# jihun1998/AO

Hardware: AMD Instinct MI355X
Metric: points/sec fwd+bwd PTv2m2 S3DIS (higher is better)
Workload: dtype fp32

## Files before the change

ao_amd/csrc/gva_wgrad_tile.hip:

```cpp
#include <algorithm>
#include <cstdlib>

#include "gva_common.h"
#include "wgrad_job.h"

namespace gva {

typedef float wt_v4f __attribute__((ext_vector_type(4)));
__device__ __forceinline__ wt_v4f wt_mfma(float a, float b, wt_v4f c) { return __builtin_amdgcn_mfma_f32_16x16x4f32(a, b, c, 0, 0, 0); }

constexpr int WT_PG = 16 * 16 + 4;

template <int G, int C, int GB, int NCW>
struct WgradTileCfg {
    static constexpr int NGW = GB / 4, QB = GB / 4, GS = G / GB, CR = C / (16 * NCW);
    static_assert(GB % 4 == 0 && GB <= 16 && G % GB == 0 && C == 8 * G && C % (16 * NCW) == 0, "blocks of groups x ranges of channels");
    static constexpr size_t lds_floats = (size_t)NCW * GB * WT_PG + 4 * 4 * 64;
};

template <int G, int C, int GB, int NCW>
__device__ __forceinline__ void wp2_wgrad_tile_body(const dense::WgradJob &J, const int bx, const int gs, const int cr, float *lds) {
    using K = WgradTileCfg<G, C, GB, NCW>;
    constexpr int NGW = K::NGW, QB = K::QB, PG = WT_PG;
    float *sA = lds;
// ... 100 lines not shown
        for (int gi = 0; gi < NGW; ++gi)
#pragma unroll
            for (int ck = 0; ck < NCW; ++ck) {
                const float *src = sA + (ck * GB + wid + 4 * gi) * PG + q * 16 + l15;
#pragma unroll
                for (int ks = 0; ks < 4; ++ks) accW[gi][ck] = wt_mfma(cur.goA[gi][ks], src[ks * 64], accW[gi][ck]);
            }
        __syncthreads();
    }
    float *rec = J.part + (size_t)bx * J.rec;
    if (q < 2) {
#pragma unroll
        for (int gi = 0; gi < NGW; ++gi)
#pragma unroll
            for (int ck = 0; ck < NCW; ++ck)
#pragma unroll
                for (int r = 0; r < 4; ++r)
                    rec[((size_t)(g0 + wid + 4 * gi) * 8 + 4 * q + r) * C + c0 + 16 * ck + l15] = accW[gi][ck][r];
    }
    if (bias_thread) rec[(size_t)G * 8 * C + o0 + tid] = bacc;
}

__global__ __launch_bounds__(256) void wp2_posrel_kernel_jobs(const dense::WgradJob *__restrict__ jobs, int njobs) {
    int j = 0;
    while (j + 1 < njobs && (long long)blockIdx.x >= jobs[j + 1].ldy) ++j;
    const dense::WgradJob &J = jobs[j];
    const long long e = ((long long)blockIdx.x - J.ldy) * 256 + threadIdx.x;
    if (e >= (long long)J.n * 16) return;
    const float *__restrict__ coord = (const float *)J.aux[0];
    const int *__restrict__ idx = (const int *)J.aux[1];
    const long long pt = e >> 4;
    const int sid = idx[e];
    const long long ss = sid >= 0 ? sid : 0;
    const float x = coord[3 * ss] - coord[3 * pt], y = coord[3 * ss + 1] - coord[3 * pt + 1], z = coord[3 * ss + 2] - coord[3 * pt + 2];
    ((float4 *)J.mX[0])[e] = sid >= 0 ? make_float4(x, y, z, 0.f) : make_float4(0.f, 0.f, 0.f, 0.f);
}

__device__ __forceinline__ void wp2_wgrad_tile_dispatch(const dense::WgradJob &J, int local, float *lds) {
    const int NS = J.chunks, GS = J.tiles;
    const int bx = local % NS, rest = local / NS, gs = rest % GS, cr = rest / GS;
    switch (J.batch) {
        case 12: wp2_wgrad_tile_body<12, 96, 12, 3>(J, bx, gs, cr, lds); break;
        case 24: wp2_wgrad_tile_body<24, 192, 12, 4>(J, bx, gs, cr, lds); break;
        case 48: wp2_wgrad_tile_body<48, 384, 12, 4>(J, bx, gs, cr, lds); break;
        default: wp2_wgrad_tile_body<64, 512, 16, 4>(J, bx, gs, cr, lds); break;
    }
}

__global__ __launch_bounds__(256, 2) void wp2_wgrad_tile_kernel(dense::WgradJob J) {
    extern __shared__ float4 wt_lds4[];
    wp2_wgrad_tile_dispatch(J, (int)blockIdx.x, (float *)wt_lds4);
}

__global__ __launch_bounds__(256, 2) void wp2_wgrad_tile_kernel_jobs(const dense::WgradJob *__restrict__ jobs, int njobs) {
    extern __shared__ float4 wt_lds4[];
    int j = 0;
    while (j + 1 < njobs && (int)blockIdx.x >= jobs[j + 1].wg0) ++j;
    const dense::WgradJob &J = jobs[j];
    wp2_wgrad_tile_dispatch(J, (int)blockIdx.x - J.wg0, (float *)wt_lds4);
}

constexpr size_t WT_LDS_BYTES = sizeof(float) * std::max({WgradTileCfg<12, 96, 12, 3>::lds_floats, WgradTileCfg<24, 192, 12, 4>::lds_floats,
                                                          WgradTileCfg<48, 384, 12, 4>::lds_floats, WgradTileCfg<64, 512, 16, 4>::lds_floats});

}

int gva_wgrad_tile_supported(int k, int c, int g) {
    return k == 16 && ((g == 12 && c == 96) || (g == 24 && c == 192) || (g == 48 && c == 384) || (g == 64 && c == 512));
}

size_t gva_wgrad_tile_plan(dense::WgradJob *J, int max_splits) {
    const int g = J->batch, c = J->cin;
    const int gb = g == 64 ? 16 : 12, ncw = g == 12 ? 3 : 4;
    const int tiles = (J->n + 15) / 16;
    J->tiles = g / gb;
    J->tiles_i = c / (16 * ncw);
    J->chunks = std::max(1, std::min({tiles / 6, 48, std::max(1, max_splits)}));
    J->chunk = (tiles + J->chunks - 1) / J->chunks * 16;
    J->rec = g * (8 * c + 8);
    J->wgs = J->chunks * J->tiles * J->tiles_i;
    J->has_pb = 1;
    J->count = 0;
    J->cout = 8;
    J->gw = gb;
    return (size_t)J->chunks * J->rec;
}

static bool wgrad_tile_configure() {
    static const bool ok = hipFuncSetAttribute((const void *)gva::wp2_wgrad_tile_kernel, hipFuncAttributeMaxDynamicSharedMemorySize,
                                               (int)gva::WT_LDS_BYTES) == hipSuccess &&
                           hipFuncSetAttribute((const void *)gva::wp2_wgrad_tile_kernel_jobs, hipFuncAttributeMaxDynamicSharedMemorySize,
                                               (int)gva::WT_LDS_BYTES) == hipSuccess;
    return ok;
}

int gva_wgrad_tile_launch_one(const dense::WgradJob &J, hipStream_t st) {
    if (!wgrad_tile_configure()) return PTV2_ERR_LAUNCH;
    hipLaunchKernelGGL(gva::wp2_wgrad_tile_kernel, dim3((unsigned)J.wgs), dim3(256), gva::WT_LDS_BYTES, st, J);
    return PTV2_OK;
}

int gva_wgrad_tile_launch_jobs(const dense::WgradJob *table, int njobs, int wgs, int pos_wgs, hipStream_t st) {
    if (!wgrad_tile_configure()) return PTV2_ERR_LAUNCH;
    if (pos_wgs > 0) hipLaunchKernelGGL(gva::wp2_posrel_kernel_jobs, dim3((unsigned)pos_wgs), dim3(256), 0, st, table, njobs);
    hipLaunchKernelGGL(gva::wp2_wgrad_tile_kernel_jobs, dim3((unsigned)wgs), dim3(256), gva::WT_LDS_BYTES, st, table, njobs);
    return PTV2_OK;
}
```

ao_amd/csrc/internal.h:

```cpp
#pragma once

struct GvaPlan;
namespace gva {
struct FoldWFwdArgs; struct FoldWBwdArgs; struct PtvDrop;
struct AttnIn; struct AttnFwdOut; struct AttnBwdIn; struct AttnBwdOut;
struct LogitsIn; struct LogitsOut; struct LogitsBwdIn; struct LogitsBwdOut;
}
namespace dense { struct WgradJob; struct BnTileSet; }

void ptv2_profile_scope(int which, int end, int ring_entry, int ring_size);
int rows_gemm_record_rows(int m, int n, int k);
void ptv2_gemm_allow_rb16(int on);
size_t bn_tiles_floats_rb(int n, int c, int rb);
int bn_tiles_finalize_rb(int n, int c, const dense::BnTileSet &S, float eps, float momentum, void *stream);
int bn_tiles_finalize_pair(int n, int c, const dense::BnTileSet (&S)[2], float eps, float momentum, void *stream);
int bn_tiles_apply_residual(int n, int c, const dense::BnTileSet &S, float eps, float momentum, const float *x,
                            const float *residual, const float *rowscale, float *y, void *stream);
int bn_tiles_apply_relu(int n, int c, const dense::BnTileSet &S, float eps, float momentum, const float *x, float *y, void *stream);
int skinny_linear_forward_pair(int n, int cin, int cout, const float *const *x, const float *W, const float *const *xsc,
                               const float *const *xsh, float *const *y, void *stream);
void ptv2_skinny_bn_arm(int n, int c, const float *const *x, const float *const *gy, const float *const *mean,
                        const float *const *rstd, const float *const *gamma, const float *const *beta, int relu, void *workspace,
                        size_t workspace_bytes);
void ptv2_skinny_bn_disarm(void);
struct PtvSkinnyBnScope {
    PtvSkinnyBnScope() = default;
    ~PtvSkinnyBnScope() { ptv2_skinny_bn_disarm(); }
    PtvSkinnyBnScope(const PtvSkinnyBnScope &) = delete;
    PtvSkinnyBnScope &operator=(const PtvSkinnyBnScope &) = delete;
};
int skinny_backward_pair_bn_reduce(int n, int cin, int cout, const float *const *gy, const float *W, float *const *gx,
                                   void *stream);
int ptv2_skinny_bn_take_records(int n, int c, const float *part, const float *const *gy);
extern "C" int linear_wgrad_strided_rowscale(int n, int cout, int cin, int batch, const float *gY, long long ldy, long long sy,
                                             const float *X, long long ldx, long long sx, float *dW, float *db,
                                             const float *rowscale, long long lds_s, int *weighted, void *workspace,
                                             size_t workspace_bytes, void *stream);
int gva_wp2_wgrad_recompute(int n, int k, int c, int g, const gva::AttnIn &I, const gva::AttnBwdIn &X, float *dW, float *db,
                            void *workspace, size_t workspace_bytes, void *stream);
int ptv2_blocks_fold_forward(int count, const ptv2_block *blocks, void *stream);
int gva_fold_forward_batched(int count, const ptv2_gva_block *blocks, void *stream);
int gva_block_forward_stats(const ptv2_gva_block *B, float *out_stats, int *stats_done, void *workspace, size_t workspace_bytes,
                            void *stream);
void ptv2_gva_set_prefolded(int on);
size_t ptv2_gva_fold_scratch_floats(int c, int g);
void ptv2_gva_set_fold_scratch(float *p);
int ptv2_gva_flush_folds(void *stream);
void ptv2_gva_drop_folds();
int gva_logits_forward_fold(const GvaPlan &P, int n, int k, int c, int g, const gva::LogitsIn &I, const gva::LogitsOut &O,
                            const gva::FoldWFwdArgs &F, void *workspace, size_t workspace_bytes, void *stream);
int gva_fwd_point_supported(int k, int c, int g);
int gva_fwd_point_max_n();
int gva_fwd_point_launch(int n, int k, int c, int g, const gva::AttnIn &I, const gva::AttnFwdOut &O, void *stream);
int gva_fwd_tile_supported(int k, int c, int g);
int gva_fwd_tile_launch(int n, int k, int c, int g, const gva::AttnIn &I, const gva::AttnFwdOut &O, void *stream);
int gva_peb_forward_stats(int n, int c, int g, const gva::AttnIn &I, const gva::AttnFwdOut &O, int *stats_done, void *stream);
int gva_aggregate_forward(const GvaPlan &P, int n, int k, int c, int g, const gva::AttnIn &I, const gva::AttnFwdOut &O,
                          void *stream);
int gva_aggregate_backward(const GvaPlan &P, int n, int k, int c, int g, const gva::AttnIn &I, const gva::AttnBwdIn &X,
                           const gva::AttnBwdOut &O, void *workspace, size_t workspace_bytes, void *stream);
int gva_logits_backward_foldw(const GvaPlan &P, int n, int k, int c, int g, const gva::LogitsIn &I, const gva::LogitsBwdIn &X,
                              const gva::FoldWBwdArgs &F, const gva::LogitsBwdOut &O, void *workspace, size_t workspace_bytes,
                              void *stream);
int gva_logits_bwd_fused_supported(int k, int c, int g);
int gva_logits_bwd_fused_launch(int n, int k, int c, int g, const gva::LogitsIn &I, const gva::LogitsBwdIn &X,
                                const gva::FoldWBwdArgs &F, float *gWt, float *part, size_t part_floats_avail,
                                const gva::LogitsBwdOut &O, hipStream_t st);
int gva_logits_fwd_mfma_supported(int k, int c, int g);
int gva_logits_fwd_mfma_launch(int n, int k, int c, int g, const gva::LogitsIn &I, const gva::LogitsOut &O, float *part,
                               const gva::FoldWFwdArgs &F, hipStream_t st);
int gva_bwd_point_supported(int k, int c, int g);
int gva_bwd_point_local(int k, int c, int g);
size_t gva_bwd_point_part_floats(int c, int g);
int gva_bwd_point_launch(int n, int k, int c, int g, const gva::AttnIn &I, const gva::AttnBwdIn &X, const gva::AttnBwdOut &O,
                         float *part, size_t part_floats_avail, hipStream_t st, gva::PtvDrop drop);
int gva_softmax_point_launch(int n, int k, int g, const gva::AttnIn &I, const gva::AttnFwdOut &O, hipStream_t st,
                             gva::PtvDrop drop);
int gva_logits_point_launch(int n, int k, int c, int g, const gva::LogitsIn &I, const gva::LogitsOut &O, float *part,
                            const gva::FoldWFwdArgs &F, hipStream_t st);
int gva_logits_params_point_launch(int n, int k, int c, int g, const gva::LogitsIn &I, const float *gWt, float *part,
                                   int max_blocks, int *nblk_out, hipStream_t st);
int gva_bwd_tile_supported(int k, int c, int g);
size_t gva_bwd_tile_part_floats(int n, int c, int g);
int gva_bwd_tile_launch(int n, int k, int c, int g, const gva::AttnIn &I, const gva::AttnBwdIn &X, const gva::AttnBwdOut &O,
                        float *part, size_t part_floats_avail, gva::PtvDrop drop, hipStream_t st);
int gva_wgrad_tile_supported(int k, int c, int g);
size_t gva_wgrad_tile_plan(dense::WgradJob *J, int max_splits);
int gva_wgrad_tile_launch_one(const dense::WgradJob &J, hipStream_t st);
int gva_wgrad_tile_launch_jobs(const dense::WgradJob *table, int njobs, int wgs, int pos_wgs, hipStream_t st);
```

ao_amd/csrc/wgrad.hip:

```cpp
#include <vector>

#include "dense_common.h"
#include "wgrad_job.h"

namespace dense {

using f32x4 = __attribute__((ext_vector_type(4))) float;
constexpr int WG_MT = 3, WG_TILE = 16 * WG_MT, WG_CHUNK = 256, WG_CHUNK_MIN = 128;

template <bool BF16>
__device__ __forceinline__ void wgrad_direct_tile(const int n, const int cout, const int cin, const int tiles_i,
                                                  const float *__restrict__ A, const long long ldy,
                                                  const float *__restrict__ B, const long long ldx, float *__restrict__ part,
                                                  const bool part_b, const int batch, const float *__restrict__ xs,
                                                  const float *__restrict__ xh, const int chunk, const int bx, const int by,
                                                  const int bz) {
    __shared__ float sRed[TPB / WAVE][WG_MT * WG_MT * 4 + WG_MT][WAVE + 1];
    const int lane = threadIdx.x & 63, wid = threadIdx.x >> 6;
    const int to = (by / tiles_i) * WG_TILE, ti = (by % tiles_i) * WG_TILE;
    const long long r0 = (long long)bx * chunk;
    const long long r1 = (r0 + chunk) < (long long)n ? (r0 + chunk) : (long long)n;
    const int lr = lane >> 4, lc = lane & 15;
    f32x4 acc[WG_MT][WG_MT];
    float bsum[WG_MT];
#pragma unroll
    for (int m = 0; m < WG_MT; ++m) {
        bsum[m] = 0.f;
#pragma unroll
        for (int t = 0; t < WG_MT; ++t) acc[m][t] = (f32x4){0.f, 0.f, 0.f, 0.f};
    }
    bool mo[WG_MT], mi[WG_MT];
    float xsc_[WG_MT], xsh_[WG_MT];
#pragma unroll
    for (int m = 0; m < WG_MT; ++m) {
        mo[m] = to + m * 16 + lc < cout;
        mi[m] = ti + m * 16 + lc < cin;
        xsc_[m] = (xs && mi[m]) ? xs[ti + m * 16 + lc] : 1.f;
        xsh_[m] = (xs && mi[m]) ? xh[ti + m * 16 + lc] : 0.f;
    }
    constexpr int U = 8;
    for (long long rb = r0 + 4 * wid; rb < r1; rb += 4 * (TPB / WAVE) * U) {
        float a[U][WG_MT], b[U][WG_MT];
#pragma unroll
        for (int u = 0; u < U; ++u) {
            const long long row = rb + (long long)u * 4 * (TPB / WAVE) + lr;
            const bool rok = row < r1;
#pragma unroll
            for (int m = 0; m < WG_MT; ++m) {
                a[u][m] = (rok && mo[m]) ? A[row * ldy + to + m * 16 + lc] : 0.f;
                b[u][m] = (rok && mi[m]) ? B[row * ldx + ti + m * 16 + lc] : 0.f;
            }
        }
        if (xs) {
#pragma unroll
            for (int u = 0; u < U; ++u)
#pragma unroll
                for (int m = 0; m < WG_MT; ++m) b[u][m] = fmaxf(__builtin_fmaf(b[u][m], xsc_[m], xsh_[m]), 0.f);
        }
        if constexpr (BF16) {
            ptv2_bf16x8 ab[WG_MT], bb[WG_MT];
#pragma unroll
            for (int m = 0; m < WG_MT; ++m) {
#pragma unroll
                for (int u = 0; u < U; ++u) {
                    bsum[m] += a[u][m];
                    ab[m][u] = (__bf16)a[u][m];
                    bb[m][u] = (__bf16)b[u][m];
                }
            }
#pragma unroll
            for (int m = 0; m < WG_MT; ++m)
#pragma unroll
                for (int t = 0; t < WG_MT; ++t)
                    acc[m][t] = __builtin_amdgcn_mfma_f32_16x16x32_bf16(ab[m], bb[t], acc[m][t], 0, 0, 0);
        } else {
#pragma unroll
            for (int u = 0; u < U; ++u)
#pragma unroll
                for (int m = 0; m < WG_MT; ++m) {
                    bsum[m] += a[u][m];
#pragma unroll
                    for (int t = 0; t < WG_MT; ++t)
                        acc[m][t] = __builtin_amdgcn_mfma_f32_16x16x4f32(a[u][m], b[u][t], acc[m][t], 0, 0, 0);
                }
        }
    }
#pragma unroll
    for (int m = 0; m < WG_MT; ++m) {
        float bs = bsum[m];
        bs += __shfl_xor(bs, 16, WAVE);
        bs += __shfl_xor(bs, 32, WAVE);
        sRed[wid][WG_MT * WG_MT * 4 + m][lane] = bs;
#pragma unroll
        for (int t = 0; t < WG_MT; ++t)
#pragma unroll
            for (int r = 0; r < 4; ++r) sRed[wid][(m * WG_MT + t) * 4 + r][lane] = acc[m][t][r];
    }
    __syncthreads();
    const size_t rec = (size_t)batch * cout * cin + (part_b ? (size_t)batch * cout : 0);
    float *p = part + (size_t)bx * rec + (size_t)bz * cout * cin;
    for (int e = threadIdx.x; e < WG_MT * WG_MT * 4 * WAVE; e += TPB) {
        const int q = e / WAVE, l = e - q * WAVE;
        const int mt = q / 4, r = q - mt * 4, m = mt / WG_MT, t = mt - m * WG_MT;
        const int o = to + m * 16 + (l >> 4) * 4 + r, i = ti + t * 16 + (l & 15);
        if (o < cout && i < cin) {
            float v = 0.f;
#pragma unroll
            for (int wv = 0; wv < TPB / WAVE; ++wv) v += sRed[wv][q][l];
            p[(size_t)o * cin + i] = v;
        }
    }
    if (part_b && ti == 0 && threadIdx.x < WG_TILE) {
        const int m = threadIdx.x >> 4, l = threadIdx.x & 15, o = to + threadIdx.x;
        if (o < cout) {
            float v = 0.f;
#pragma unroll
            for (int wv = 0; wv < TPB / WAVE; ++wv) v += sRed[wv][WG_MT * WG_MT * 4 + m][l];
            part[(size_t)bx * rec + (size_t)batch * cout * cin + (size_t)bz * cout + o] = v;
        }
    }
}

template <bool BF16>
__device__ __forceinline__ void wgrad_direct_job(const WgradJob &J, const int bx, const int by, const int bz) {
    const bool multi = J.count > 0;
    wgrad_direct_tile<BF16>(J.n, J.cout, J.cin, J.tiles_i, multi ? J.mgY[bz] : J.gY + (long long)bz * J.sy, J.ldy,
                            multi ? J.mX[bz] : J.X + (long long)bz * J.sx, J.ldx, J.part, J.has_pb != 0, J.batch,
                            multi ? J.mxsc[bz] : nullptr, multi ? J.mxsh[bz] : nullptr, J.chunk, bx, by, bz);
}
template <bool BF16>
__global__ __launch_bounds__(TPB) void linear_wgrad_kernel(WgradJob J) {
    wgrad_direct_job<BF16>(J, (int)blockIdx.x, (int)blockIdx.y, (int)blockIdx.z);
}

constexpr int WL_ROWS = 64;
template <int RS>
__device__ __forceinline__ void wgrad_lds_tile(const int n, const int cout, const int cin, const int tiles_i,
                                               const float *__restrict__ A, const long long ldy,
                                               const float *__restrict__ B, const long long ldx,
                                               float *__restrict__ part, const bool part_b, const int batch,
                                               const float *__restrict__ xs, const float *__restrict__ xh, const int chunk,
                                               const float *__restrict__ rowscale, const long long lds_s, const int bx,
                                               const int by, const int bz) {
    extern __shared__ float4 wl_lds4[];
    float *sA = (float *)wl_lds4;
    float *sB = sA + 2 * WL_ROWS * WG_TILE;
    const int tid = threadIdx.x, lane = tid & 63, wid = tid >> 6;
    const int to = (by / tiles_i) * WG_TILE, ti = (by % tiles_i) * WG_TILE;
    const long long r0 = (long long)bx * chunk;
    const long long r1 = (r0 + chunk) < (long long)n ? (r0 + chunk) : (long long)n;
    const int lr = lane >> 4, lc = lane & 15;
    f32x4 acc[WG_MT][WG_MT];
    float bsum[WG_MT];
#pragma unroll
    for (int m = 0; m < WG_MT; ++m) {
        bsum[m] = 0.f;
#pragma unroll
        for (int t = 0; t < WG_MT; ++t) acc[m][t] = (f32x4){0.f, 0.f, 0.f, 0.f};
    }
    float xsc_[WG_MT], xsh_[WG_MT];
#pragma unroll
    for (int m = 0; m < WG_MT; ++m) {
        const bool mi = ti + m * 16 + lc < cin;
        xsc_[m] = (xs && mi) ? xs[ti + m * 16 + lc] : 1.f;
        xsh_[m] = (xs && mi) ? xh[ti + m * 16 + lc] : 0.f;
    }
    constexpr int Q = WG_TILE / 4, SLOTS = WL_ROWS * Q / TPB;
    float4 ra[SLOTS], rb[SLOTS];
    float sn[4], sc_[4];
    auto fetch = [&](long long rs) {
#pragma unroll
        for (int j = 0; j < SLOTS; ++j) {
            const int f = tid + TPB * j, row = f / Q, c4 = (f - row * Q) * 4;
            const long long r = rs + row;
            ra[j] = ptv2_ld_or_zero((const float4 *)(A + r * ldy + to + c4), r < r1 && to + c4 < cout);
            rb[j] = ptv2_ld_or_zero((const float4 *)(B + r * ldx + ti + c4), r < r1 && ti + c4 < cin);
        }
        if constexpr (RS != 0) {
#pragma unroll
            for (int ks = 0; ks < 4; ++ks) {
                const long long r = rs + wid * 16 + ks * 4 + lr;
                sn[ks] = ptv2_ld_or_zero(rowscale + r * lds_s + bz, r < r1);
            }
        }
    };
// ... 51 lines not shown
        bs += __shfl_xor(bs, 16, WAVE);
        bs += __shfl_xor(bs, 32, WAVE);
        sRed[wid][WG_MT * WG_MT * 4 + m][lane] = bs;
#pragma unroll
        for (int t = 0; t < WG_MT; ++t)
#pragma unroll
            for (int r = 0; r < 4; ++r) sRed[wid][(m * WG_MT + t) * 4 + r][lane] = acc[m][t][r];
    }
    __syncthreads();
    const size_t rec = (size_t)batch * cout * cin + (part_b ? (size_t)batch * cout : 0);
    float *p = part + (size_t)bx * rec + (size_t)bz * cout * cin;
    for (int e = threadIdx.x; e < WG_MT * WG_MT * 4 * WAVE; e += TPB) {
        const int q = e / WAVE, l = e - q * WAVE;
        const int mt = q / 4, r = q - mt * 4, m = mt / WG_MT, t = mt - m * WG_MT;
        const int o = to + m * 16 + (l >> 4) * 4 + r, i = ti + t * 16 + (l & 15);
        if (o < cout && i < cin) {
            float v = 0.f;
#pragma unroll
            for (int wv = 0; wv < TPB / WAVE; ++wv) v += sRed[wv][q][l];
            p[(size_t)o * cin + i] = v;
        }
    }
    if (part_b && ti == 0 && threadIdx.x < WG_TILE) {
        const int m = threadIdx.x >> 4, l = threadIdx.x & 15, o = to + threadIdx.x;
        if (o < cout) {
            float v = 0.f;
#pragma unroll
            for (int wv = 0; wv < TPB / WAVE; ++wv) v += sRed[wv][WG_MT * WG_MT * 4 + m][l];
            part[(size_t)bx * rec + (size_t)batch * cout * cin + (size_t)bz * cout + o] = v;
        }
    }
}

template <int RS>
__device__ __forceinline__ void wgrad_lds_job(const WgradJob &J, const int bx, const int by, const int bz) {
    const bool multi = J.count > 0;
    wgrad_lds_tile<RS>(J.n, J.cout, J.cin, J.tiles_i, multi ? J.mgY[bz] : J.gY + (long long)bz * J.sy, J.ldy,
                       multi ? J.mX[bz] : J.X + (long long)bz * J.sx, J.ldx, J.part, J.has_pb != 0, J.batch,
                       multi ? J.mxsc[bz] : nullptr, multi ? J.mxsh[bz] : nullptr, J.chunk, J.rowscale, J.lds_s, bx, by, bz);
}
template <int RS>
__global__ __launch_bounds__(TPB) void linear_wgrad_lds_kernel(WgradJob J) {
    wgrad_lds_job<RS>(J, (int)blockIdx.x, (int)blockIdx.y, (int)blockIdx.z);
}

constexpr int WGRAD_PACK = 8;
struct WgradJobPack { WgradJob j[WGRAD_PACK]; };
static_assert(sizeof(WgradJobPack) + 16 <= 4096, "the table writer's argument block must fit the 4 KB kernarg segment");
__global__ void wgrad_jobs_write_kernel(WgradJobPack pack, int count, WgradJob *table) {
    if ((int)threadIdx.x < count) table[threadIdx.x] = pack.j[threadIdx.x];
}

template <int RS>
__global__ __launch_bounds__(TPB) void linear_wgrad_lds_kernel_jobs(const WgradJob *__restrict__ jobs, int njobs) {
    int j = 0;
    while (j + 1 < njobs && (int)blockIdx.x >= jobs[j + 1].wg0) ++j;
    const WgradJob &J = jobs[j];
    const int local = (int)blockIdx.x - J.wg0;
    const int rest = local / J.chunks;
    wgrad_lds_job<RS>(J, local % J.chunks, rest % J.tiles, rest / J.tiles);
}

constexpr int GRP_I = 8;
__device__ __forceinline__ void grouped_wgrad_tile(const int n, const int c, const int g, const int gw, const int chunk,
                                                   const float *__restrict__ gY, const float *__restrict__ X,
                                                   const float *__restrict__ sw, float *__restrict__ part, const int rec,
                                                   const int bx, const int bg) {
    extern __shared__ float4 grp_lds4[];
    const int q = c >> 2, units = gw * q, R = max(1, TPB / units);
    const int tid = threadIdx.x, rs = tid / units, u = tid - rs * units;
    const bool active = rs < R;
    const int gl = u / q, qi = u - gl * q, grp = bg * gw + gl;
    const bool live = active && grp < g;
    float4 acc[GRP_I];
    float bacc[GRP_I];
#pragma unroll
    for (int i = 0; i < GRP_I; ++i) { acc[i] = make_float4(0.f, 0.f, 0.f, 0.f); bacc[i] = 0.f; }
    const long long r0 = (long long)bx * chunk, r1 = (r0 + chunk) < (long long)n ? (r0 + chunk) : (long long)n;
    if (live) {
        const float *xa = X + (size_t)grp * c + 4 * qi;
        const float *ya = gY + (size_t)grp * GRP_I;
        const float *sa = sw + grp;
        const size_t xs = (size_t)g * c;
        constexpr int U = 4;
        long long r = r0 + rs;
        for (; r + (long long)(U - 1) * R < r1; r += (long long)U * R) {
            float4 a[U], y0[U], y1[U];
            float s[U];
#pragma unroll
            for (int t = 0; t < U; ++t) {
                const size_t rr = (size_t)(r + (long long)t * R);
                a[t] = *(const float4 *)(xa + rr * xs);
                y0[t] = *(const float4 *)(ya + rr * c);
                y1[t] = *(const float4 *)(ya + rr * c + 4);
                s[t] = qi == 0 ? sa[rr * g] : 0.f;
            }
#pragma unroll
            for (int t = 0; t < U; ++t) {
                const float y[GRP_I] = {y0[t].x, y0[t].y, y0[t].z, y0[t].w, y1[t].x, y1[t].y, y1[t].z, y1[t].w};
#pragma unroll
                for (int i = 0; i < GRP_I; ++i) {
                    acc[i].x = __builtin_fmaf(y[i], a[t].x, acc[i].x); acc[i].y = __builtin_fmaf(y[i], a[t].y, acc[i].y);
                    acc[i].z = __builtin_fmaf(y[i], a[t].z, acc[i].z); acc[i].w = __builtin_fmaf(y[i], a[t].w, acc[i].w);
                    bacc[i] = __builtin_fmaf(y[i], s[t], bacc[i]);
                }
            }
        }
        for (; r < r1; r += R) {
            const size_t rr = (size_t)r;
            const float4 a = *(const float4 *)(xa + rr * xs), y0 = *(const float4 *)(ya + rr * c), y1 = *(const float4 *)(ya + rr * c + 4);
            const float sv = qi == 0 ? sa[rr * g] : 0.f;
            const float y[GRP_I] = {y0.x, y0.y, y0.z, y0.w, y1.x, y1.y, y1.z, y1.w};
#pragma unroll
            for (int i = 0; i < GRP_I; ++i) {
                acc[i].x = __builtin_fmaf(y[i], a.x, acc[i].x); acc[i].y = __builtin_fmaf(y[i], a.y, acc[i].y);
                acc[i].z = __builtin_fmaf(y[i], a.z, acc[i].z); acc[i].w = __builtin_fmaf(y[i], a.w, acc[i].w);
                bacc[i] = __builtin_fmaf(y[i], sv, bacc[i]);
            }
        }
    }
    float4 *sAcc = grp_lds4;
    float *sB = (float *)(sAcc + (size_t)R * GRP_I * units);
    if (active) {
#pragma unroll
        for (int i = 0; i < GRP_I; ++i) {
            sAcc[((size_t)rs * GRP_I + i) * units + u] = acc[i];
            if (qi == 0) sB[((size_t)rs * GRP_I + i) * gw + gl] = bacc[i];
        }
    }
    __syncthreads();
    if (rs == 0 && grp < g) {
        float *p = part + (size_t)bx * rec;
#pragma unroll
        for (int i = 0; i < GRP_I; ++i) {
            float4 v = sAcc[(size_t)i * units + u];
            for (int t = 1; t < R; ++t) {
                const float4 w = sAcc[((size_t)t * GRP_I + i) * units + u];
                v.x += w.x; v.y += w.y; v.z += w.z; v.w += w.w;
            }
            *(float4 *)(p + ((size_t)grp * GRP_I + i) * c + 4 * qi) = v;
            if (qi == 0) {
                float b = sB[(size_t)i * gw + gl];
                for (int t = 1; t < R; ++t) b += sB[((size_t)t * GRP_I + i) * gw + gl];
                p[(size_t)g * GRP_I * c + (size_t)grp * GRP_I + i] = b;
            }
        }
    }
}
inline size_t grouped_lds_bytes(int c, int gw) {
    const int units = gw * (c >> 2), R = std::max(1, TPB / units);
    return sizeof(float4) * (size_t)R * GRP_I * units + sizeof(float) * (size_t)R * GRP_I * gw;
}
__global__ __launch_bounds__(TPB) void grouped_wgrad_kernel(WgradJob J) {
    const int bx = (int)blockIdx.x % J.chunks, bg = (int)blockIdx.x / J.chunks;
    grouped_wgrad_tile(J.n, J.cin, J.batch, J.gw, J.chunk, J.gY, J.X, J.rowscale, J.part, J.rec, bx, bg);
}
__global__ __launch_bounds__(TPB) void grouped_wgrad_kernel_jobs(const WgradJob *__restrict__ jobs, int njobs) {
    int j = 0;
    while (j + 1 < njobs && (int)blockIdx.x >= jobs[j + 1].wg0) ++j;
    const WgradJob &J = jobs[j];
    const int local = (int)blockIdx.x - J.wg0;
    grouped_wgrad_tile(J.n, J.cin, J.batch, J.gw, J.chunk, J.gY, J.X, J.rowscale, J.part, J.rec, local % J.chunks, local / J.chunks);
}

template <bool BF16>
__global__ __launch_bounds__(TPB) void linear_wgrad_kernel_jobs(const WgradJob *__restrict__ jobs, int njobs) {
    int j = 0;
    while (j + 1 < njobs && (int)blockIdx.x >= jobs[j + 1].wg0) ++j;
    const WgradJob &J = jobs[j];
    const int local = (int)blockIdx.x - J.wg0;
    const int rest = local / J.chunks;
    wgrad_direct_job<BF16>(J, local % J.chunks, rest % J.tiles, rest / J.tiles);
}

__global__ __launch_bounds__(256) void wgrad_jobs_finalize_kernel(const WgradJob *__restrict__ jobs, int njobs, int total) {
    __shared__ double s_sum[3][64];
    const int sidx = blockIdx.x * 256 + threadIdx.x;
    int j = 0;
    while (j + 1 < njobs && (int)blockIdx.x * 256 >= jobs[j + 1].fin0) ++j;
    const WgradJob &J = jobs[j];
    const int lanes = J.fin_lanes, local = sidx - J.fin0;
    const int rg = lanes == 1 ? 0 : (int)threadIdx.x >> 6;
    const int col = lanes == 1 ? local : (local >> 8) * 64 + ((int)threadIdx.x & 63);
    const int nblk = J.chunks;
    const size_t len = (size_t)J.rec;
    const float *part = J.part;
    const bool ok = col < J.rec;
    double a0 = 0.0, a1 = 0.0, a2 = 0.0, a3 = 0.0;
    if (ok) {
        int b = rg;
        for (; b + 3 * lanes < nblk; b += 4 * lanes) {
            a0 += (double)part[(size_t)b * len + col];
            a1 += (double)part[(size_t)(b + lanes) * len + col];
            a2 += (double)part[(size_t)(b + 2 * lanes) * len + col];
            a3 += (double)part[(size_t)(b + 3 * lanes) * len + col];
        }
        for (; b < nblk; b += lanes) a0 += (double)part[(size_t)b * len + col];
    }
    double acc = (a0 + a1) + (a2 + a3);
    if (lanes != 1) {
        if (rg > 0) s_sum[rg - 1][threadIdx.x & 63] = acc;
        __syncthreads();
        if (rg > 0) return;
        acc = (acc + s_sum[0][threadIdx.x]) + (s_sum[1][threadIdx.x] + s_sum[2][threadIdx.x]);
    }
    if (!ok) return;
    const float v = (float)acc;
    const int wlen = J.cout * J.cin, wtot = J.batch * wlen;
    if (J.count > 0) {
        if (col < wtot) {
            const int p = col / wlen;
            J.mdW[p][col - p * wlen] = v;
        } else {
            const int r = col - wtot, p = r / J.cout;
            if (J.mdb[p]) J.mdb[p][r - p * J.cout] = v;
        }
    } else if (col < wtot) {
        J.dW[col] = v;
    } else if (J.db) {
        J.db[col - wtot] = v;
    }
}

static bool wgrad_lds_ok(const void *a, long long ldy, long long sy, const void *b, long long ldx, long long sx) {
    return ((uintptr_t)a % 16 == 0) && ((uintptr_t)b % 16 == 0) && ldy % 4 == 0 && ldx % 4 == 0 && sy % 4 == 0 && sx % 4 == 0;
}
static bool wgrad_lds_shape_ok(int cout, int cin) { return cout % 4 == 0 && cin % 4 == 0; }
constexpr size_t WL_LDS_BYTES = sizeof(float) * std::max<size_t>(4 * (size_t)WL_ROWS * WG_TILE,
                                                                 (size_t)(TPB / WAVE) * (WG_MT * WG_MT * 4 + WG_MT) * (WAVE + 1));

}

using namespace dense;

extern "C" size_t dense_workspace_bytes(int n, int cout, int cin) {
    const size_t chunks = (size_t)(n + WG_CHUNK_MIN - 1) / WG_CHUNK_MIN + 1;
    const size_t wg = sizeof(float) * chunks * ((size_t)cout * cin + cout);
    const size_t bn = sizeof(float) * (size_t)MAX_BLK * 2 * (size_t)std::max(cout, cin);
    return ptv2_align256(std::max(wg, bn)) + 1024;
}

static int wg_chunk(int n, int tiles, bool filed = false) {
    const int target = filed ? 256 : 768;
    const int chunks = std::max(1, target / std::max(1, tiles));
    const long long rows = ((long long)n + chunks - 1) / chunks;
    long long chunk = std::max<long long>(WG_CHUNK, (rows + 127) / 128 * 128);
    if (tiles > 1) {
        int guard = 0;
        while ((((long long)n + chunk - 1) / chunk) % 8 == 0 && ((long long)n + chunk - 1) / chunk > 1 && guard++ < 16) chunk += 128;
    }
    return (int)std::min<long long>(chunk, 1 << 20);
}

namespace {
enum WgradForm { WF_LDS = 0, WF_LDS_RS, WF_DIRECT, WF_DIRECT_BF16, WF_GROUPED, WF_RECOMPUTE, WGRAD_FORMS };
constexpr int wgrad_kid(WgradForm f) {
    return f == WF_RECOMPUTE ? KID_WGRAD_TILE : f == WF_GROUPED ? KID_WGRAD_GROUPED : (f == WF_LDS || f == WF_LDS_RS) ? KID_WGRAD_LDS : KID_WGRAD;
}
struct WgradCall {
    WgradJob J;
    WgradForm form;
    double bytes;
    size_t posrel;
};

struct WgradDefer {
    bool active = false;
    bool armed = false;
    bool armed_rs = false;
    char *arena = nullptr;
    size_t cap = 0, used = 0;
    std::vector<WgradJob> jobs[WGRAD_FORMS];
    double bytes[WGRAD_FORMS] = {};
};
thread_local WgradDefer g_wdefer;
constexpr int WGRAD_MAX_JOBS = 64;
constexpr size_t WGRAD_TABLE_BYTES = ptv2_align256(sizeof(WgradJob) * WGRAD_MAX_JOBS);

bool may_file(bool rs) { return g_wdefer.active && (rs ? g_wdefer.armed_rs : g_wdefer.armed); }

bool wgrad_configure() {
    static const bool ok = [] {
        const void *kernels[4] = {(const void *)linear_wgrad_lds_kernel<0>, (const void *)linear_wgrad_lds_kernel<1>,
                                  (const void *)linear_wgrad_lds_kernel_jobs<0>, (const void *)linear_wgrad_lds_kernel_jobs<1>};
        bool all = true;
        for (const void *k : kernels)
            all = hipFuncSetAttribute(k, hipFuncAttributeMaxDynamicSharedMemorySize, (int)WL_LDS_BYTES) == hipSuccess && all;
        return all;
    }();
    return ok;
}
}

void ptv2_wgrad_defer_begin(void *arena, size_t bytes) {
    WgradDefer &D = g_wdefer;
    for (int f = 0; f < WGRAD_FORMS; ++f) { D.jobs[f].clear(); D.bytes[f] = 0.0; }
    D.armed = D.armed_rs = false;
    D.active = arena != nullptr && bytes > WGRAD_FORMS * WGRAD_TABLE_BYTES;
    D.arena = (char *)arena;
    D.cap = bytes;
    D.used = WGRAD_FORMS * WGRAD_TABLE_BYTES;
}
bool ptv2_wgrad_defer_active() { return g_wdefer.active; }
void ptv2_wgrad_defer_end() {
    g_wdefer.active = g_wdefer.armed = g_wdefer.armed_rs = false;
    for (auto &j : g_wdefer.jobs) j.clear();
}
void ptv2_wgrad_defer_arm(bool on) { g_wdefer.armed = on && g_wdefer.active; }
void ptv2_wgrad_defer_arm_rs(bool on) { g_wdefer.armed_rs = on && g_wdefer.active; }
bool ptv2_wgrad_defer_armed_rs() { return may_file(true); }
size_t ptv2_wgrad_defer_table_bytes() { return WGRAD_FORMS * WGRAD_TABLE_BYTES; }
float *ptv2_wgrad_defer_alloc(size_t floats) {
    WgradDefer &D = g_wdefer;
    const size_t bytes = ptv2_align256(sizeof(float) * floats);
    if (!D.active || D.used + bytes > D.cap) return nullptr;
    float *p = (float *)(D.arena + D.used);
    D.used += bytes;
    return p;
}
int ptv2_wgrad_defer_flush(void *stream) {
    WgradDefer &D = g_wdefer;
    if (!D.active) return PTV2_OK;
    hipStream_t st = (hipStream_t)stream;
    if (!wgrad_configure()) return PTV2_ERR_LAUNCH;
    for (int f = 0; f < WGRAD_FORMS; ++f) {
        const WgradForm form = (WgradForm)f;
        std::vector<WgradJob> &jobs = D.jobs[form];
        if (jobs.empty()) continue;
        WgradJob *table = (WgradJob *)(D.arena + (size_t)form * WGRAD_TABLE_BYTES);
        const int njobs = (int)jobs.size();
        const bool row_pieces = form == WF_GROUPED || form == WF_RECOMPUTE;
        std::stable_sort(jobs.begin(), jobs.end(), [row_pieces](const WgradJob &a, const WgradJob &b) {
            const long long wa = (long long)a.chunk * (row_pieces ? a.gw * a.cin : 1), wb = (long long)b.chunk * (row_pieces ? b.gw * b.cin : 1);
            return wa > wb;
        });
        int wgs = 0, fin = 0;
        long long pos_wgs = 0;
        bool pos_all = form == WF_RECOMPUTE;
        for (WgradJob &J : jobs) {
            if (form == WF_RECOMPUTE) {
                J.ldy = pos_wgs;
                pos_wgs += ((long long)J.n * 16 + 255) / 256;
                pos_all = pos_all && J.mX[0] != nullptr;
            }
            J.wg0 = wgs; J.fin0 = fin;
            J.fin_lanes = J.chunks > 32 ? 4 : 1;
            wgs += J.wgs;
            fin += J.fin_lanes == 1 ? (J.rec + 255) / 256 * 256 : (J.rec + 63) / 64 * 256;
        }
        for (int at = 0; at < njobs; at += WGRAD_PACK) {
            WgradJobPack pack;
            const int cnt = std::min(WGRAD_PACK, njobs - at);
            for (int i = 0; i < WGRAD_PACK; ++i) pack.j[i] = jobs[(size_t)std::min(at + i, njobs - 1)];
            hipLaunchKernelGGL(wgrad_jobs_write_kernel, dim3(1), dim3(64), 0, st, pack, cnt, table + at);
        }
        {
            PtvScopedTimer t(wgrad_kid(form), st, D.bytes[form]);
            const dim3 grid((unsigned)wgs), block(TPB);
            const WgradJob *tab = table;
            switch (form) {
                case WF_LDS: hipLaunchKernelGGL(linear_wgrad_lds_kernel_jobs<0>, grid, block, WL_LDS_BYTES, st, tab, njobs); break;
                case WF_LDS_RS: hipLaunchKernelGGL(linear_wgrad_lds_kernel_jobs<1>, grid, block, WL_LDS_BYTES, st, tab, njobs); break;
                case WF_DIRECT: hipLaunchKernelGGL(linear_wgrad_kernel_jobs<false>, grid, block, 0, st, tab, njobs); break;
                case WF_DIRECT_BF16: hipLaunchKernelGGL(linear_wgrad_kernel_jobs<true>, grid, block, 0, st, tab, njobs); break;
                case WF_GROUPED: {
                    size_t lds = 0;
                    for (const WgradJob &J : jobs) lds = std::max(lds, grouped_lds_bytes(J.cin, J.gw));
                    hipLaunchKernelGGL(grouped_wgrad_kernel_jobs, grid, block, lds, st, tab, njobs);
                    break;
                }
                default:
                    if (gva_wgrad_tile_launch_jobs(tab, njobs, wgs, pos_all ? (int)pos_wgs : 0, st) != PTV2_OK) return PTV2_ERR_LAUNCH;
            }
        }
        hipLaunchKernelGGL(wgrad_jobs_finalize_kernel, dim3((unsigned)((fin + 255) / 256)), dim3(256), 0, st,
                           (const WgradJob *)table, njobs, fin);
        jobs.clear();
        D.bytes[form] = 0.0;
    }
    PTV2_CHECK_LAUNCH();
    return PTV2_OK;
}

struct MapWgradMulti {
    float *dW[6], *db[6];
    int count, wlen, cout;
    explicit MapWgradMulti(const WgradJob &J) : count(J.count), wlen(J.cout * J.cin), cout(J.cout) {
        for (int i = 0; i < 6; ++i) { dW[i] = J.mdW[i]; db[i] = J.mdb[i]; }
    }
    __device__ void operator()(int e, double v) const {
        const int wtot = count * wlen;
        if (e < wtot) {
            const int b = e / wlen;
            dW[b][e - b * wlen] = (float)v;
        } else {
            const int r = e - wtot, b = r / cout;
            if (db[b]) db[b][r - b * cout] = (float)v;
        }
    }
};

namespace gva {
template <> struct RiderOf<MapWgradMulti> {
    static constexpr bool ok = true;
    static PtvRider make(const MapWgradMulti &m) {
        PtvRider r{};
        r.kind = RIDER_WGRADN;
        for (int i = 0; i < 6; ++i) { r.p[i] = i < m.count ? m.dW[i] : nullptr; r.p[6 + i] = i < m.count ? m.db[i] : nullptr; }
        r.i0 = m.wlen; r.i1 = m.cout; r.i2 = m.count;
        return r;
    }
};
}

static int wgrad_submit(WgradCall &C, bool file, void *workspace, size_t workspace_bytes, void *stream) {
    WgradDefer &D = g_wdefer;
    WgradJob &J = C.J;
    if (file && (int)D.jobs[C.form].size() < WGRAD_MAX_JOBS) {
        float *keep = ptv2_wgrad_defer_alloc((size_t)J.chunks * J.rec);
        float *pos = keep && C.posrel ? ptv2_wgrad_defer_alloc(C.posrel) : nullptr;
        if (keep && (pos || !C.posrel)) {
            J.part = keep;
            if (pos) J.mX[0] = pos;
            D.jobs[C.form].push_back(J);
            D.bytes[C.form] += C.bytes;
            return PTV2_OK;
        }
    }
    const size_t fit = workspace ? workspace_bytes / (sizeof(float) * (size_t)J.rec) : 0;
    if (C.form == WF_RECOMPUTE && fit >= 1 && fit < (size_t)J.chunks) (void)gva_wgrad_tile_plan(&J, (int)fit);
    if (fit < (size_t)J.chunks) return PTV2_ERR_WORKSPACE;
// ... 179 lines not shown
```

ao_amd/csrc/wgrad_job.h:

```cpp
#pragma once

namespace dense {

struct WgradJob {
    int n, cout, cin, tiles_i, tiles, batch, chunk, chunks;
    int wg0;
    int has_pb, count;
    int rec, fin0;
    int wgs, gw;
    int fin_lanes;
    long long ldy, sy, ldx, sx, lds_s;
    const float *gY, *X, *rowscale;
    float *part;
    const float *mgY[6], *mX[6], *mxsc[6], *mxsh[6];
    float *dW, *db, *mdW[6], *mdb[6];
    const void *aux[4];
};

}
```

Baseline: 12.84 million.

## Fold previous form's wgrad finalize blocks into next form's wgrad launch

When several wgrad forms are flushed, the finalize reduction for one form is prepended as extra blocks to the next form's wgrad kernel grid instead of being a separate launch. All job tables are written up front so the carried finalize can read them, and LDS is shared between the finalize and main paths. This cuts kernel launches and lets the small reduction overlap with the next GEMM-like work. The cost is a larger grid, an extra branch per block and more complex plan bookkeeping. It is gated by an env var (on by default) and a block-count cap.

```diff
diff --git a/ao_amd/csrc/gva_wgrad_tile.hip b/ao_amd/csrc/gva_wgrad_tile.hip
--- a/ao_amd/csrc/gva_wgrad_tile.hip
+++ b/ao_amd/csrc/gva_wgrad_tile.hip
@@ -176,12 +176,15 @@
     wp2_wgrad_tile_dispatch(J, (int)blockIdx.x, (float *)wt_lds4);
 }
 
-__global__ __launch_bounds__(256, 2) void wp2_wgrad_tile_kernel_jobs(const dense::WgradJob *__restrict__ jobs, int njobs) {
+__global__ __launch_bounds__(256, 2) void wp2_wgrad_tile_kernel_jobs(const dense::WgradJob *__restrict__ jobs, int njobs,
+                                                                     dense::WgradRide R) {
     extern __shared__ float4 wt_lds4[];
+    if (dense::wgrad_ride_block(R, (int)blockIdx.x, wt_lds4)) return;
+    const int bid = (int)blockIdx.x - R.fin_blocks;
     int j = 0;
-    while (j + 1 < njobs && (int)blockIdx.x >= jobs[j + 1].wg0) ++j;
+    while (j + 1 < njobs && bid >= jobs[j + 1].wg0) ++j;
     const dense::WgradJob &J = jobs[j];
-    wp2_wgrad_tile_dispatch(J, (int)blockIdx.x - J.wg0, (float *)wt_lds4);
+    wp2_wgrad_tile_dispatch(J, bid - J.wg0, (float *)wt_lds4);
 }
 
 constexpr size_t WT_LDS_BYTES = sizeof(float) * std::max({WgradTileCfg<12, 96, 12, 3>::lds_floats, WgradTileCfg<24, 192, 12, 4>::lds_floats,
@@ -224,9 +227,11 @@
     return PTV2_OK;
 }
 
-int gva_wgrad_tile_launch_jobs(const dense::WgradJob *table, int njobs, int wgs, int pos_wgs, hipStream_t st) {
+int gva_wgrad_tile_launch_jobs(const dense::WgradJob *table, int njobs, int wgs, int pos_wgs, const dense::WgradRide &R,
+                               hipStream_t st) {
     if (!wgrad_tile_configure()) return PTV2_ERR_LAUNCH;
     if (pos_wgs > 0) hipLaunchKernelGGL(gva::wp2_posrel_kernel_jobs, dim3((unsigned)pos_wgs), dim3(256), 0, st, table, njobs);
-    hipLaunchKernelGGL(gva::wp2_wgrad_tile_kernel_jobs, dim3((unsigned)wgs), dim3(256), gva::WT_LDS_BYTES, st, table, njobs);
+    hipLaunchKernelGGL(gva::wp2_wgrad_tile_kernel_jobs, dim3((unsigned)(R.fin_blocks + wgs)), dim3(256), gva::WT_LDS_BYTES, st, table,
+                       njobs, R);
     return PTV2_OK;
 }
diff --git a/ao_amd/csrc/internal.h b/ao_amd/csrc/internal.h
--- a/ao_amd/csrc/internal.h
+++ b/ao_amd/csrc/internal.h
@@ -6,7 +6,7 @@
 struct AttnIn; struct AttnFwdOut; struct AttnBwdIn; struct AttnBwdOut;
 struct LogitsIn; struct LogitsOut; struct LogitsBwdIn; struct LogitsBwdOut;
 }
-namespace dense { struct WgradJob; struct BnTileSet; }
+namespace dense { struct WgradJob; struct WgradRide; struct BnTileSet; }
 
 void ptv2_profile_scope(int which, int end, int ring_entry, int ring_size);
 int rows_gemm_record_rows(int m, int n, int k);
@@ -87,4 +87,4 @@
 int gva_wgrad_tile_supported(int k, int c, int g);
 size_t gva_wgrad_tile_plan(dense::WgradJob *J, int max_splits);
 int gva_wgrad_tile_launch_one(const dense::WgradJob &J, hipStream_t st);
-int gva_wgrad_tile_launch_jobs(const dense::WgradJob *table, int njobs, int wgs, int pos_wgs, hipStream_t st);
+int gva_wgrad_tile_launch_jobs(const dense::WgradJob *table, int njobs, int wgs, int pos_wgs, const dense::WgradRide &R, hipStream_t st);
diff --git a/ao_amd/csrc/wgrad.hip b/ao_amd/csrc/wgrad.hip
--- a/ao_amd/csrc/wgrad.hip
+++ b/ao_amd/csrc/wgrad.hip
@@ -7,6 +7,7 @@
 
 using f32x4 = __attribute__((ext_vector_type(4))) float;
 constexpr int WG_MT = 3, WG_TILE = 16 * WG_MT, WG_CHUNK = 256, WG_CHUNK_MIN = 128;
+typedef float WgRed[WG_MT * WG_MT * 4 + WG_MT][WAVE + 1];
 
 template <bool BF16>
 __device__ __forceinline__ void wgrad_direct_tile(const int n, const int cout, const int cin, const int tiles_i,
@@ -14,8 +15,7 @@
                                                   const float *__restrict__ B, const long long ldx, float *__restrict__ part,
                                                   const bool part_b, const int batch, const float *__restrict__ xs,
                                                   const float *__restrict__ xh, const int chunk, const int bx, const int by,
-                                                  const int bz) {
-    __shared__ float sRed[TPB / WAVE][WG_MT * WG_MT * 4 + WG_MT][WAVE + 1];
+                                                  const int bz, WgRed *sRed) {
     const int lane = threadIdx.x & 63, wid = threadIdx.x >> 6;
     const int to = (by / tiles_i) * WG_TILE, ti = (by % tiles_i) * WG_TILE;
     const long long r0 = (long long)bx * chunk;
@@ -122,15 +122,16 @@
 }
 
 template <bool BF16>
-__device__ __forceinline__ void wgrad_direct_job(const WgradJob &J, const int bx, const int by, const int bz) {
+__device__ __forceinline__ void wgrad_direct_job(const WgradJob &J, const int bx, const int by, const int bz, WgRed *sRed) {
     const bool multi = J.count > 0;
     wgrad_direct_tile<BF16>(J.n, J.cout, J.cin, J.tiles_i, multi ? J.mgY[bz] : J.gY + (long long)bz * J.sy, J.ldy,
                             multi ? J.mX[bz] : J.X + (long long)bz * J.sx, J.ldx, J.part, J.has_pb != 0, J.batch,
-                            multi ? J.mxsc[bz] : nullptr, multi ? J.mxsh[bz] : nullptr, J.chunk, bx, by, bz);
+                            multi ? J.mxsc[bz] : nullptr, multi ? J.mxsh[bz] : nullptr, J.chunk, bx, by, bz, sRed);
 }
 template <bool BF16>
 __global__ __launch_bounds__(TPB) void linear_wgrad_kernel(WgradJob J) {
-    wgrad_direct_job<BF16>(J, (int)blockIdx.x, (int)blockIdx.y, (int)blockIdx.z);
+    __shared__ __attribute__((aligned(16))) WgRed sRed[TPB / WAVE];
+    wgrad_direct_job<BF16>(J, (int)blockIdx.x, (int)blockIdx.y, (int)blockIdx.z, sRed);
 }
 
 constexpr int WL_ROWS = 64;
@@ -288,11 +289,14 @@
 }
 
 template <int RS>
-__global__ __launch_bounds__(TPB) void linear_wgrad_lds_kernel_jobs(const WgradJob *__restrict__ jobs, int njobs) {
+__global__ __launch_bounds__(TPB) void linear_wgrad_lds_kernel_jobs(const WgradJob *__restrict__ jobs, int njobs, WgradRide R) {
+    extern __shared__ float4 wl_lds4[];
+    if (wgrad_ride_block(R, (int)blockIdx.x, wl_lds4)) return;
+    const int bid = (int)blockIdx.x - R.fin_blocks;
     int j = 0;
-    while (j + 1 < njobs && (int)blockIdx.x >= jobs[j + 1].wg0) ++j;
+    while (j + 1 < njobs && bid >= jobs[j + 1].wg0) ++j;
     const WgradJob &J = jobs[j];
-    const int local = (int)blockIdx.x - J.wg0;
+    const int local = bid - J.wg0;
     const int rest = local / J.chunks;
     wgrad_lds_job<RS>(J, local % J.chunks, rest % J.tiles, rest / J.tiles);
 }
@@ -391,72 +395,35 @@
     const int bx = (int)blockIdx.x % J.chunks, bg = (int)blockIdx.x / J.chunks;
     grouped_wgrad_tile(J.n, J.cin, J.batch, J.gw, J.chunk, J.gY, J.X, J.rowscale, J.part, J.rec, bx, bg);
 }
-__global__ __launch_bounds__(TPB) void grouped_wgrad_kernel_jobs(const WgradJob *__restrict__ jobs, int njobs) {
+__global__ __launch_bounds__(TPB) void grouped_wgrad_kernel_jobs(const WgradJob *__restrict__ jobs, int njobs, WgradRide R) {
+    extern __shared__ float4 grp_lds4[];
+    if (wgrad_ride_block(R, (int)blockIdx.x, grp_lds4)) return;
+    const int bid = (int)blockIdx.x - R.fin_blocks;
     int j = 0;
-    while (j + 1 < njobs && (int)blockIdx.x >= jobs[j + 1].wg0) ++j;
+    while (j + 1 < njobs && bid >= jobs[j + 1].wg0) ++j;
     const WgradJob &J = jobs[j];
-    const int local = (int)blockIdx.x - J.wg0;
+    const int local = bid - J.wg0;
     grouped_wgrad_tile(J.n, J.cin, J.batch, J.gw, J.chunk, J.gY, J.X, J.rowscale, J.part, J.rec, local % J.chunks, local / J.chunks);
 }
 
 template <bool BF16>
-__global__ __launch_bounds__(TPB) void linear_wgrad_kernel_jobs(const WgradJob *__restrict__ jobs, int njobs) {
+__global__ __launch_bounds__(TPB) void linear_wgrad_kernel_jobs(const WgradJob *__restrict__ jobs, int njobs, WgradRide R) {
+    __shared__ __attribute__((aligned(16))) WgRed sRed[TPB / WAVE];
+    if (wgrad_ride_block(R, (int)blockIdx.x, sRed)) return;
+    const int bid = (int)blockIdx.x - R.fin_blocks;
     int j = 0;
-    while (j + 1 < njobs && (int)blockIdx.x >= jobs[j + 1].wg0) ++j;
+    while (j + 1 < njobs && bid >= jobs[j + 1].wg0) ++j;
     const WgradJob &J = jobs[j];
-    const int local = (int)blockIdx.x - J.wg0;
+    const int local = bid - J.wg0;
     const int rest = local / J.chunks;
-    wgrad_direct_job<BF16>(J, local % J.chunks, rest % J.tiles, rest / J.tiles);
+    wgrad_direct_job<BF16>(J, local % J.chunks, rest % J.tiles, rest / J.tiles, sRed);
 }
 
 __global__ __launch_bounds__(256) void wgrad_jobs_finalize_kernel(const WgradJob *__restrict__ jobs, int njobs, int total) {
-    __shared__ double s_sum[3][64];
-    const int sidx = blockIdx.x * 256 + threadIdx.x;
-    int j = 0;
-    while (j + 1 < njobs && (int)blockIdx.x * 256 >= jobs[j + 1].fin0) ++j;
-    const WgradJob &J = jobs[j];
-    const int lanes = J.fin_lanes, local = sidx - J.fin0;
-    const int rg = lanes == 1 ? 0 : (int)threadIdx.x >> 6;
-    const int col = lanes == 1 ? local : (local >> 8) * 64 + ((int)threadIdx.x & 63);
-    const int nblk = J.chunks;
-    const size_t len = (size_t)J.rec;
-    const float *part = J.part;
-    const bool ok = col < J.rec;
-    double a0 = 0.0, a1 = 0.0, a2 = 0.0, a3 = 0.0;
-    if (ok) {
-        int b = rg;
-        for (; b + 3 * lanes < nblk; b += 4 * lanes) {
-            a0 += (double)part[(size_t)b * len + col];
-            a1 += (double)part[(size_t)(b + lanes) * len + col];
-            a2 += (double)part[(size_t)(b + 2 * lanes) * len + col];
-            a3 += (double)part[(size_t)(b + 3 * lanes) * len + col];
-        }
-        for (; b < nblk; b += lanes) a0 += (double)part[(size_t)b * len + col];
-    }
-    double acc = (a0 + a1) + (a2 + a3);
-    if (lanes != 1) {
-        if (rg > 0) s_sum[rg - 1][threadIdx.x & 63] = acc;
-        __syncthreads();
-        if (rg > 0) return;
-        acc = (acc + s_sum[0][threadIdx.x]) + (s_sum[1][threadIdx.x] + s_sum[2][threadIdx.x]);
-    }
-    if (!ok) return;
-    const float v = (float)acc;
-    const int wlen = J.cout * J.cin, wtot = J.batch * wlen;
-    if (J.count > 0) {
-        if (col < wtot) {
-            const int p = col / wlen;
-            J.mdW[p][col - p * wlen] = v;
-        } else {
-            const int r = col - wtot, p = r / J.cout;
-            if (J.mdb[p]) J.mdb[p][r - p * J.cout] = v;
-        }
-    } else if (col < wtot) {
-        J.dW[col] = v;
-    } else if (J.db) {
-        J.db[col - wtot] = v;
-    }
-}
+    __shared__ double s_sum[3 * 64];
+    wgrad_jobs_finalize_block(jobs, njobs, (int)blockIdx.x, s_sum);
+}
+constexpr size_t WGRAD_RIDE_LDS = sizeof(double) * 3 * 64;
 
 static bool wgrad_lds_ok(const void *a, long long ldy, long long sy, const void *b, long long ldx, long long sx) {
     return ((uintptr_t)a % 16 == 0) && ((uintptr_t)b % 16 == 0) && ldy % 4 == 0 && ldx % 4 == 0 && sy % 4 == 0 && sx % 4 == 0;
@@ -554,17 +521,27 @@
     D.used += bytes;
     return p;
 }
+constexpr int WGRAD_RIDE_MAX_BLOCKS = 256;
 int ptv2_wgrad_defer_flush(void *stream) {
     WgradDefer &D = g_wdefer;
     if (!D.active) return PTV2_OK;
     hipStream_t st = (hipStream_t)stream;
     if (!wgrad_configure()) return PTV2_ERR_LAUNCH;
+    const bool ride = !ptv2_env_is("AO_AMD_WGRAD_RIDE", '0');
+    struct Plan {
+        WgradJob *table;
+        int njobs, wgs, fin;
+        int pos_wgs;
+    } plan[WGRAD_FORMS] = {};
+    int order[WGRAD_FORMS], nforms = 0;
     for (int f = 0; f < WGRAD_FORMS; ++f) {
         const WgradForm form = (WgradForm)f;
         std::vector<WgradJob> &jobs = D.jobs[form];
         if (jobs.empty()) continue;
-        WgradJob *table = (WgradJob *)(D.arena + (size_t)form * WGRAD_TABLE_BYTES);
-        const int njobs = (int)jobs.size();
+        order[nforms++] = f;
+        Plan &P = plan[f];
+        P.table = (WgradJob *)(D.arena + (size_t)form * WGRAD_TABLE_BYTES);
+        P.njobs = (int)jobs.size();
         const bool row_pieces = form == WF_GROUPED || form == WF_RECOMPUTE;
         std::stable_sort(jobs.begin(), jobs.end(), [row_pieces](const WgradJob &a, const WgradJob &b) {
             const long long wa = (long long)a.chunk * (row_pieces ? a.gw * a.cin : 1), wb = (long long)b.chunk * (row_pieces ? b.gw * b.cin : 1);
@@ -584,35 +561,61 @@
             wgs += J.wgs;
             fin += J.fin_lanes == 1 ? (J.rec + 255) / 256 * 256 : (J.rec + 63) / 64 * 256;
         }
+        P.wgs = wgs; P.fin = fin;
+        P.pos_wgs = pos_all ? (int)pos_wgs : 0;
+    }
+    auto write_table = [&](int f) {
+        const std::vector<WgradJob> &jobs = D.jobs[f];
+        const int njobs = plan[f].njobs;
         for (int at = 0; at < njobs; at += WGRAD_PACK) {
             WgradJobPack pack;
             const int cnt = std::min(WGRAD_PACK, njobs - at);
             for (int i = 0; i < WGRAD_PACK; ++i) pack.j[i] = jobs[(size_t)std::min(at + i, njobs - 1)];
-            hipLaunchKernelGGL(wgrad_jobs_write_kernel, dim3(1), dim3(64), 0, st, pack, cnt, table + at);
+            hipLaunchKernelGGL(wgrad_jobs_write_kernel, dim3(1), dim3(64), 0, st, pack, cnt, plan[f].table + at);
+        }
+    };
+    if (ride)
+        for (int k = 0; k < nforms; ++k) write_table(order[k]);
+    int rc = PTV2_OK;
+    bool carried = false;
+    for (int k = 0; k < nforms && rc == PTV2_OK; ++k) {
+        const int f = order[k];
+        const WgradForm form = (WgradForm)f;
+        const Plan &P = plan[f];
+        if (!ride) write_table(f);
+        WgradRide R{};
+        if (carried) {
+            const Plan &Q = plan[order[k - 1]];
+            R.fin_jobs = Q.table; R.fin_njobs = Q.njobs; R.fin_blocks = Q.fin / 256;
         }
         {
             PtvScopedTimer t(wgrad_kid(form), st, D.bytes[form]);
-            const dim3 grid((unsigned)wgs), block(TPB);
-            const WgradJob *tab = table;
+            const dim3 grid((unsigned)(R.fin_blocks + P.wgs)), block(TPB);
+            const WgradJob *tab = P.table;
+            const int njobs = P.njobs;
             switch (form) {
-                case WF_LDS: hipLaunchKernelGGL(linear_wgrad_lds_kernel_jobs<0>, grid, block, WL_LDS_BYTES, st, tab, njobs); break;
-                case WF_LDS_RS: hipLaunchKernelGGL(linear_wgrad_lds_kernel_jobs<1>, grid, block, WL_LDS_BYTES, st, tab, njobs); break;
-                case WF_DIRECT: hipLaunchKernelGGL(linear_wgrad_kernel_jobs<false>, grid, block, 0, st, tab, njobs); break;
-                case WF_DIRECT_BF16: hipLaunchKernelGGL(linear_wgrad_kernel_jobs<true>, grid, block, 0, st, tab, njobs); break;
+                case WF_LDS: hipLaunchKernelGGL(linear_wgrad_lds_kernel_jobs<0>, grid, block, WL_LDS_BYTES, st, tab, njobs, R); break;
+                case WF_LDS_RS: hipLaunchKernelGGL(linear_wgrad_lds_kernel_jobs<1>, grid, block, WL_LDS_BYTES, st, tab, njobs, R); break;
+                case WF_DIRECT: hipLaunchKernelGGL(linear_wgrad_kernel_jobs<false>, grid, block, 0, st, tab, njobs, R); break;
+                case WF_DIRECT_BF16: hipLaunchKernelGGL(linear_wgrad_kernel_jobs<true>, grid, block, 0, st, tab, njobs, R); break;
                 case WF_GROUPED: {
-                    size_t lds = 0;
-                    for (const WgradJob &J : jobs) lds = std::max(lds, grouped_lds_bytes(J.cin, J.gw));
-                    hipLaunchKernelGGL(grouped_wgrad_kernel_jobs, grid, block, lds, st, tab, njobs);
+                    size_t lds = WGRAD_RIDE_LDS;
+                    for (const WgradJob &J : D.jobs[f]) lds = std::max(lds, grouped_lds_bytes(J.cin, J.gw));
+                    hipLaunchKernelGGL(grouped_wgrad_kernel_jobs, grid, block, lds, st, tab, njobs, R);
                     break;
                 }
-                default:
-                    if (gva_wgrad_tile_launch_jobs(tab, njobs, wgs, pos_all ? (int)pos_wgs : 0, st) != PTV2_OK) return PTV2_ERR_LAUNCH;
-            }
-        }
-        hipLaunchKernelGGL(wgrad_jobs_finalize_kernel, dim3((unsigned)((fin + 255) / 256)), dim3(256), 0, st,
-                           (const WgradJob *)table, njobs, fin);
-        jobs.clear();
-        D.bytes[form] = 0.0;
+                default: rc = gva_wgrad_tile_launch_jobs(tab, njobs, P.wgs, P.pos_wgs, R, st);
+            }
+        }
+        carried = ride && k + 1 < nforms && P.fin / 256 <= WGRAD_RIDE_MAX_BLOCKS;
+        if (rc == PTV2_OK && !carried)
+            hipLaunchKernelGGL(wgrad_jobs_finalize_kernel, dim3((unsigned)(P.fin / 256)), dim3(256), 0, st, (const WgradJob *)P.table,
+                               P.njobs, P.fin);
+    }
+    if (rc != PTV2_OK) return rc;
+    for (int k = 0; k < nforms; ++k) {
+        D.jobs[order[k]].clear();
+        D.bytes[order[k]] = 0.0;
     }
     PTV2_CHECK_LAUNCH();
     return PTV2_OK;
diff --git a/ao_amd/csrc/wgrad_job.h b/ao_amd/csrc/wgrad_job.h
--- a/ao_amd/csrc/wgrad_job.h
+++ b/ao_amd/csrc/wgrad_job.h
@@ -17,4 +17,64 @@
     const void *aux[4];
 };
 
+struct WgradRide {
+    const WgradJob *fin_jobs;
+    int fin_njobs, fin_blocks;
+};
+
+__device__ __forceinline__ void wgrad_jobs_finalize_block(const WgradJob *__restrict__ jobs, const int njobs, const int block,
+                                                          double *s_sum) {
+    const int sidx = block * 256 + threadIdx.x;
+    int j = 0;
+    while (j + 1 < njobs && block * 256 >= jobs[j + 1].fin0) ++j;
+    const WgradJob &J = jobs[j];
+    const int lanes = J.fin_lanes, local = sidx - J.fin0;
+    const int rg = lanes == 1 ? 0 : (int)threadIdx.x >> 6;
+    const int col = lanes == 1 ? local : (local >> 8) * 64 + ((int)threadIdx.x & 63);
+    const int nblk = J.chunks;
+    const size_t len = (size_t)J.rec;
+    const float *part = J.part;
+    const bool ok = col < J.rec;
+    double a0 = 0.0, a1 = 0.0, a2 = 0.0, a3 = 0.0;
+    if (ok) {
+        int b = rg;
+        for (; b + 3 * lanes < nblk; b += 4 * lanes) {
+            a0 += (double)part[(size_t)b * len + col];
+            a1 += (double)part[(size_t)(b + lanes) * len + col];
+            a2 += (double)part[(size_t)(b + 2 * lanes) * len + col];
+            a3 += (double)part[(size_t)(b + 3 * lanes) * len + col];
+        }
+        for (; b < nblk; b += lanes) a0 += (double)part[(size_t)b * len + col];
+    }
+    double acc = (a0 + a1) + (a2 + a3);
+    if (lanes != 1) {
+        if (rg > 0) s_sum[(rg - 1) * 64 + (threadIdx.x & 63)] = acc;
+        __syncthreads();
+        if (rg > 0) return;
+        acc = (acc + s_sum[threadIdx.x]) + (s_sum[64 + threadIdx.x] + s_sum[128 + threadIdx.x]);
+    }
+    if (!ok) return;
+    const float v = (float)acc;
+    const int wlen = J.cout * J.cin, wtot = J.batch * wlen;
+    if (J.count > 0) {
+        if (col < wtot) {
+            const int p = col / wlen;
+            J.mdW[p][col - p * wlen] = v;
+        } else {
+            const int r = col - wtot, p = r / J.cout;
+            if (J.mdb[p]) J.mdb[p][r - p * J.cout] = v;
+        }
+    } else if (col < wtot) {
+        J.dW[col] = v;
+    } else if (J.db) {
+        J.db[col - wtot] = v;
+    }
 }
+
+__device__ __forceinline__ bool wgrad_ride_block(const WgradRide &R, const int block, void *lds) {
+    if (block >= R.fin_blocks) return false;
+    wgrad_jobs_finalize_block(R.fin_jobs, R.fin_njobs, block, (double *)lds);
+    return true;
+}
+
+}
```

Result: no change. 12.88 million (median of 6 runs) (+0.3%).
